# Ezreal11/EaBNet

Measured on AMD Instinct MI355X. Metric: enhanced frames/sec (16 kHz, 8-mic) at 1/2/4/8 MI355X; RTF per utterance, higher is better.
Workload: dtype f32; 1 GPU; BASELINE configs[1]/[2]: batch of 16 four-second 8-mic 16 kHz utterances per GPU, wave -> STFT+compress -> EaBNet.forward, inference, full hand-written HIP path; batch_per_gpu=16, global_batch=16, mics=8, frames_per_utt=401, freq_bins=161, parallelism=dp1 (independent shards, no collective), pipeline_depth=3

## Files before the change

### eabnet_amd/csrc/conv_gemm.hip

```cpp
#include "device.h"
#include <type_traits>

#define CG_THREADS 256

#define CG_PLAIN 0
#define CG_GLU 1
#define CG_DUAL 2
#define CG_PH2 3
#define CG_XFC 128

#define CG_PMAX 352

template <int MI, int NI, int KU, int MODE, bool PATCH, bool XFT>
struct CgSmem {
    static constexpr int BM = 64 * MI, BN = 64 * NI, LDK = 16 * KU + 4;
    static constexpr int NA = MODE == CG_DUAL ? 2 : 1;
    static constexpr int ATILE = BM * LDK;
    float a[PATCH ? CG_PMAX * LDK : NA * 2 * ATILE];
    float b[2][BN * LDK];
    float xft[2][CG_XFC][2];
    float xsl[2][CG_XFC];
    int dt[EAB_MAX_TAPS];
    int ioff[EAB_MAX_TAPS];
    int last;
    static constexpr int RW = MODE == CG_PH2 ? 2 : 1;
    __attribute__((aligned(16))) unsigned rtab_own[XFT ? BM * RW : 4];
    static_assert(XFT || sizeof(float) * 2 * CG_XFC * 2 >= sizeof(unsigned) * BM * RW, "row table inside xft");
};

__device__ __forceinline__ void cg_merge(float& n, float& mean, float& m2, float nb, float meanb, float m2b) {
    const float nt = n + nb;
    if (nt > 0.0f) {
        const float delta = meanb - mean;
        const float fb = nb / nt;
        mean = fmaf(delta, fb, mean);
        m2 = m2 + m2b + delta * delta * n * fb;
    }
    n = nt;
}

template <int MI, int NI, int KU, int MODE, int XF, bool VEC, int PREC, bool PATCH, bool WIDE = false>
__global__ __launch_bounds__(CG_THREADS, (MI == 2 && NI == 2 && KU == 1 && MODE == CG_GLU) ? 3 : (MODE == CG_PH2 ? 2 : 1)) void conv_gemm_kernel(const eab_conv_desc d) {
    static_assert(MODE != CG_PH2 || (PATCH && NI == 2), "phase-pair form: patch pipeline, one column block per phase and wave");
    static_assert(!PATCH || (KU == 1 && MODE != CG_DUAL && VEC), "patch mode: one unit per stage, single transform");
    constexpr bool H3 = PREC == EAB_PREC_F16X3;
    constexpr bool BF = PREC == EAB_PREC_BF16;
    constexpr bool PH2 = MODE == CG_PH2;
    constexpr bool GLU = MODE != CG_PLAIN;
    constexpr bool DUAL = MODE == CG_DUAL;
    using Smem = CgSmem<MI, NI, KU, MODE, PATCH, XF != EAB_XF_NONE>;
    constexpr int BM = Smem::BM, BN = Smem::BN, LDK = Smem::LDK;
    __shared__ __attribute__((aligned(16))) Smem sm;

    const int tid = threadIdx.x;
    const int lane = tid & 63, wave = tid >> 6;
    const int wm = wave >> 1, wn = wave & 1;
    const int li = lane & 31, lh = lane >> 5;

    const int t_lo = d.win.pos ? *d.win.pos : 0;
    int t_hi = d.win.pos ? (t_lo + d.win.count < d.T ? t_lo + d.win.count : d.T) : d.T;
    const int tiles_per_b = ((d.win.pos ? d.win.count : d.T) * d.No + BM - 1) / BM;
    unsigned vblk = blockIdx.x;
    if (gridDim.x >= 64) {
        const unsigned G = gridDim.x, G8 = G >> 3, rem = G & 7, xcd = vblk & 7, idx = vblk >> 3;
        vblk = xcd * G8 + (xcd < rem ? xcd : rem) + idx;
    }
    const int b = (int)(vblk / (unsigned)tiles_per_b);
    const int tile = (int)vblk - b * tiles_per_b;
    int t_src = d.T;
    if (d.win.lens) {
        t_src = min(t_src, d.win.lens[b]);
        t_hi = min(t_hi, t_src);
    }
    const int Q = t_hi * d.No;
    const int q0 = t_lo * d.No + tile * BM;
    const int n_blk = blockIdx.y * BN;
    const float inv_no = 1.0f / (float)d.No;

#pragma unroll
    for (int j = 0; j < EAB_MAX_TAPS; ++j)
        if (tid == j) {
            sm.dt[j] = d.dt[j];
            sm.ioff[j] = d.ioff[j];
        }

    const int Cout = d.Cout;
    const unsigned row_bytes = (unsigned)(d.Fout * Cout) * 4u, step_bytes = (unsigned)(d.ostride * Cout) * 4u;
    const unsigned phase_bytes = (unsigned)(d.ophase * Cout) * 4u, chan_bytes = (unsigned)Cout * 4u;
    unsigned* const rtab = XF != EAB_XF_NONE ? sm.rtab_own : reinterpret_cast<unsigned*>(&sm.xft[0][0][0]);
    if (tid < BM) {
        const int q = q0 + tid;
        const bool ok = q < Q;
        const int t = eab_div(ok ? q : 0, d.No, inv_no), o = (ok ? q : 0) - t * d.No;
        const unsigned off = ok ? (unsigned)t * row_bytes + (unsigned)o * step_bytes + phase_bytes : EAB_OOB;
        if constexpr (PH2)
            *reinterpret_cast<uint2*>(&rtab[2 * tid]) = make_uint2(off, (ok && 2 * o + 1 < d.Fout) ? off + chan_bytes : EAB_OOB);
        else
            rtab[tid] = off;
    }

    if (XF != EAB_XF_NONE) {
        const int k = tid >> 7, c = tid & (CG_XFC - 1);
        const int Ck = (k == 0 || DUAL) ? d.C0 : d.C1;
        const float* xfk = k == 0 ? d.xf0 : d.xf1;
        const float* slk = k == 0 ? d.slope0 : d.slope1;
        float sc = 1.0f, sh = 0.0f, sl = 1.0f;
        if (c < Ck) {
            if (d.fin_stats && k < d.fin_nsets) {
                const float* gm = k == 0 ? d.fin_gamma0 : d.fin_gamma1;
                const float* bt = k == 0 ? d.fin_beta0 : d.fin_beta1;
                double sn = 0.0, sm = 0.0, sq = 0.0;
                for (int t = 0; t < d.fin_tiles; ++t) {
                    const f32x4 v = *reinterpret_cast<const f32x4*>(
                        &d.fin_stats[((((size_t)b * d.fin_tiles + t) * d.fin_nsets + k) * d.C0 + c) * 4]);
                    const double n = (double)v[0], mu = (double)v[1];
                    sn += n;
                    sm = fma(n, mu, sm);
                    sq += fma(n * mu, mu, (double)v[2]);
                }
                const double mean = sn > 0.0 ? sm / sn : 0.0;
                double var = sn > 0.0 ? sq / sn - mean * mean : 0.0;
                if (var < 0.0) var = 0.0;
                const double scale = (double)gm[c] / sqrt(var + (double)d.fin_eps);
                sc = (float)scale;
                sh = (float)((double)bt[c] - mean * scale);
                sl = slk[c];
            } else if (xfk) {
                const float2 v = *reinterpret_cast<const float2*>(&xfk[((size_t)b * Ck + c) * 2]);
                sc = v.x;
                sh = v.y;
                sl = slk[c];
            }
        }
        sm.xft[k][c][0] = sc;
        sm.xft[k][c][1] = sh;
        sm.xsl[k][c] = sl;
    }

    const int Ctot = d.C0 + d.C1;
    const int UPT = (Ctot + 15) >> 4;
    const int NU = d.ntaps * UPT;
    static_assert(!WIDE || (PREC == EAB_PREC_BF16 && KU == 1 && VEC && !PATCH && XF == EAB_XF_NONE && MODE != CG_DUAL), "WIDE: see above");
    constexpr bool w0 = WIDE, w1 = WIDE;
    const int NS = (w0 || w1) ? d.ntaps * ((w0 ? d.C0 >> 5 : (d.C0 + 15) >> 4) + (d.C1 > 0 ? (w1 ? d.C1 >> 5 : (d.C1 + 15) >> 4) : 0))
                              : (NU + KU - 1) / KU;

    constexpr unsigned esz0 = WIDE ? 2u : 4u, esz1 = WIDE ? 2u : 4u;
    const unsigned bytes0 = (unsigned)d.T * d.Fin * d.C0 * esz0;
    const unsigned bytes1 = (unsigned)d.T * d.Fin * d.C1 * esz1;
    const __amdgpu_buffer_rsrc_t rs0 = __builtin_amdgcn_make_buffer_rsrc(
        const_cast<char*>(reinterpret_cast<const char*>(d.src0)) + (size_t)b * bytes0, 0, bytes0, 0x00020000);
    const __amdgpu_buffer_rsrc_t rs1 = __builtin_amdgcn_make_buffer_rsrc(
        const_cast<char*>(reinterpret_cast<const char*>(d.src1 ? d.src1 : d.src0)) + (d.src1 ? (size_t)b * bytes1 : 0), 0,
        d.src1 ? bytes1 : 0u, 0x00020000);

    const int srow = tid >> 2;
    const int skq = tid & 3;
    const float* wrow[NI];
#pragma unroll
    for (int p = 0; p < NI; ++p) wrow[p] = d.w + (size_t)(n_blk + srow + 64 * p) * d.Kpad + skq * 4;

    f32x16 acc[MI][NI];
#pragma unroll
    for (int mi = 0; mi < MI; ++mi)
#pragma unroll
        for (int ni = 0; ni < NI; ++ni)
#pragma unroll
            for (int r = 0; r < 16; ++r) acc[mi][ni][r] = 0.0f;

    auto lds_barrier = [] { asm volatile("s_waitcnt lgkmcnt(0)\n\ts_barrier" ::: "memory"); };

    __syncthreads();

    if (q0 < Q) {
    if constexpr (PATCH) {
        constexpr int PP = (CG_PMAX + 63) / 64;
        int dt_min = 0, io_min = 0, io_max = 0;
#pragma unroll
        for (int j = 0; j < EAB_MAX_TAPS; ++j)
            if (j < d.ntaps) {
                dt_min = d.dt[j] < dt_min ? d.dt[j] : dt_min;
                io_min = d.ioff[j] < io_min ? d.ioff[j] : io_min;
                io_max = d.ioff[j] > io_max ? d.ioff[j] : io_max;
            }
        const int halo_lo = -io_min;
        const int hi_need = (d.No - 1) * d.istride + io_max - (d.Fin - 1);
        const int Fp = d.Fin + halo_lo + (hi_need > 0 ? hi_need : 0);
        const float inv_fp = 1.0f / (float)Fp;
        const int t_first = eab_div(q0, d.No, inv_no);
        const int t_last = eab_div((q0 + BM < Q ? q0 + BM : (Q > q0 ? Q : q0 + 1)) - 1, d.No, inv_no);
        const int P = (t_last - t_first + 1 - dt_min) * Fp;

        const int d64 = eab_div(64, Fp, inv_fp), m64 = 64 - d64 * Fp;
        int p_tf[PP];
        bool p_ok[PP], p_all[PP];
        {
            const int tr = eab_div(srow, Fp, inv_fp);
            int f = srow - tr * Fp, t_in = t_first + dt_min + tr;
            int tf = t_in * d.Fin + f - halo_lo;
#pragma unroll
            for (int pp = 0; pp < PP; ++pp) {
                p_ok[pp] = p_all[pp] = false;
                p_tf[pp] = 0;
                if (64 * pp < P) {
                    p_ok[pp] = srow + 64 * pp < P && (unsigned)t_in < (unsigned)t_src && (unsigned)(f - halo_lo) < (unsigned)d.Fin;
                    if (XF != EAB_XF_NONE) p_all[pp] = __builtin_amdgcn_ballot_w64(p_ok[pp]) == __builtin_amdgcn_ballot_w64(true);
                    p_tf[pp] = tf;
                    f += m64;
                    t_in += d64;
                    tf += d64 * d.Fin + m64;
                    if (f >= Fp) {
                        f -= Fp;
                        ++t_in;
                        tf += d.Fin - Fp;
                    }
                }
            }
        }
        int fa[MI];
#pragma unroll
        for (int mi = 0; mi < MI; ++mi) {
            int q = q0 + (wm * MI + mi) * 32 + li;
            q = q < Q ? q : (Q > q0 ? Q - 1 : q0);
            const int t = eab_div(q, d.No, inv_no), o = q - t * d.No;
            fa[mi] = ((t - t_first - dt_min) * Fp + o * d.istride + halo_lo) * LDK + 4 * lh;
        }
        const int b_base = (wn * NI * 32 + li) * LDK + 4 * lh;

        f32x4 rp[PP];
        f32x4 rbw0[NI], rbw1[NI];
        int p_tc = 0;
        auto patch_fetch = [&](int chunk) {
            const int c0 = chunk << 4;
            const bool second = (d.C1 > 0) && (c0 >= d.C0);
            const int Cs = second ? d.C1 : d.C0;
            const int c = (second ? c0 - d.C0 : c0) + skq * 4;
            const bool cok = c < Cs;
            p_tc = ((second ? 1 : 0) << 8) | (cok ? c : 0);
#pragma unroll
            for (int pp = 0; pp < PP; ++pp) {
                if (64 * pp >= P) continue;
                const unsigned off = (p_ok[pp] && cok) ? (unsigned)((p_tf[pp] * Cs + c) * 4) : EAB_OOB;
                const u32x4 v = second ? __builtin_amdgcn_raw_buffer_load_b128(rs1, off, 0, 0)
                                       : __builtin_amdgcn_raw_buffer_load_b128(rs0, off, 0, 0);
                rp[pp] = __builtin_bit_cast(f32x4, v);
            }
        };
        auto patch_stash = [&]() {
            f32x4 sh01, sh23, sl;
            if (XF != EAB_XF_NONE) {
                const int cc = p_tc & 0xFF, tb = p_tc >> 8;
                sh01 = *reinterpret_cast<const f32x4*>(&sm.xft[tb][cc][0]);
                sh23 = *reinterpret_cast<const f32x4*>(&sm.xft[tb][cc + 2][0]);
                sl = *reinterpret_cast<const f32x4*>(&sm.xsl[tb][cc]);
            }
#pragma unroll
            for (int pp = 0; pp < PP; ++pp) {
                const int pidx = srow + 64 * pp;
                if (pidx >= CG_PMAX) continue;
                if (64 * pp >= P) continue;
                f32x4 v = rp[pp];
                if (XF != EAB_XF_NONE) {
                    const f32x4 x = eab_xform<XF>(v, sh01, sh23, sl);
                    v = x;
                    if (!p_all[pp]) {
                        asm volatile("; rim" ::: "memory");
                        v = p_ok[pp] ? x : f32x4{0.f, 0.f, 0.f, 0.f};
                    }
                }
                float* arow = &sm.a[pidx * LDK];
                if (BF) {
                    *reinterpret_cast<uint2*>(reinterpret_cast<char*>(arow) + skq * 8) = make_uint2(eab_bf2(v[0], v[1]), eab_bf2(v[2], v[3]));
                } else if (H3) {
                    unsigned h01, l01, h23, l23;
                    eab_split2(v[0], v[1], h01, l01);
                    eab_split2(v[2], v[3], h23, l23);
                    *reinterpret_cast<uint2*>(reinterpret_cast<char*>(arow) + skq * 8) = make_uint2(h01, h23);
                    *reinterpret_cast<uint2*>(reinterpret_cast<char*>(arow) + 32 + skq * 8) = make_uint2(l01, l23);
                } else {
                    *reinterpret_cast<f32x4*>(arow + skq * 4) = v;
                }
            }
        };
        auto b_fetch = [&](int u, f32x4 (&rbw)[NI]) {
            const int uu = u < NU ? u : 0;
#pragma unroll
            for (int p = 0; p < NI; ++p) rbw[p] = *reinterpret_cast<const f32x4*>(wrow[p] + (size_t)uu * 16);
        };
        auto b_stash = [&](int buf, const f32x4 (&rbw)[NI]) {
#pragma unroll
            for (int p = 0; p < NI; ++p) {
                float* brow = &sm.b[buf][(srow + 64 * p) * LDK];
                if (BF) {
                    *reinterpret_cast<uint2*>(reinterpret_cast<char*>(brow) + skq * 8) =
                        make_uint2(eab_bf2(rbw[p][0], rbw[p][1]), eab_bf2(rbw[p][2], rbw[p][3]));
                } else if (H3) {
                    const u32x4 w = __builtin_bit_cast(u32x4, rbw[p]);
                    *reinterpret_cast<uint2*>(reinterpret_cast<char*>(brow) + skq * 8) = make_uint2(w[0], w[1]);
                    *reinterpret_cast<uint2*>(reinterpret_cast<char*>(brow) + 32 + skq * 8) = make_uint2(w[2], w[3]);
                } else {
                    *reinterpret_cast<f32x4*>(brow + skq * 4) = rbw[p];
                }
            }
        };
        auto pcompute_n = [&](int cur, int tap, auto ne_c) {
            constexpr int NE = decltype(ne_c)::value;
            const int toff = (sm.dt[tap] * Fp + sm.ioff[tap]) * LDK;
            if (BF) {
                bf16x8 ab[MI], bb[NE];
#pragma unroll
                for (int mi = 0; mi < MI; ++mi) ab[mi] = *reinterpret_cast<const bf16x8*>(&sm.a[fa[mi] + toff]);
#pragma unroll
                for (int ni = 0; ni < NE; ++ni) bb[ni] = *reinterpret_cast<const bf16x8*>(&sm.b[cur][b_base + ni * 32 * LDK]);
#pragma unroll
                for (int mi = 0; mi < MI; ++mi)
#pragma unroll
                    for (int ni = 0; ni < NE; ++ni)
                        acc[mi][ni] = __builtin_amdgcn_mfma_f32_32x32x16_bf16(ab[mi], bb[ni], acc[mi][ni], 0, 0, 0);
            } else if (H3) {
                h16x8 ah[MI], al[MI], bh[NE], bl[NE];
#pragma unroll
                for (int mi = 0; mi < MI; ++mi) {
                    const char* pa = reinterpret_cast<const char*>(&sm.a[fa[mi] + toff]);
                    ah[mi] = *reinterpret_cast<const h16x8*>(pa);
                    al[mi] = *reinterpret_cast<const h16x8*>(pa + 32);
                }
#pragma unroll
                for (int ni = 0; ni < NE; ++ni) {
                    const char* pb = reinterpret_cast<const char*>(&sm.b[cur][b_base + ni * 32 * LDK]);
                    bh[ni] = *reinterpret_cast<const h16x8*>(pb);
                    bl[ni] = *reinterpret_cast<const h16x8*>(pb + 32);
                }
#pragma unroll
                for (int mi = 0; mi < MI; ++mi)
#pragma unroll
                    for (int ni = 0; ni < NE; ++ni) {
                        acc[mi][ni] = __builtin_amdgcn_mfma_f32_32x32x16_f16(al[mi], bh[ni], acc[mi][ni], 0, 0, 0);
                        acc[mi][ni] = __builtin_amdgcn_mfma_f32_32x32x16_f16(ah[mi], bl[ni], acc[mi][ni], 0, 0, 0);
                        acc[mi][ni] = __builtin_amdgcn_mfma_f32_32x32x16_f16(ah[mi], bh[ni], acc[mi][ni], 0, 0, 0);
                    }
            } else {
#pragma unroll
                for (int g = 0; g < 2; ++g) {
                    f32x4 af[MI], bf[NE];
#pragma unroll
                    for (int mi = 0; mi < MI; ++mi) af[mi] = *reinterpret_cast<const f32x4*>(&sm.a[fa[mi] + toff + g * 8]);
#pragma unroll
                    for (int ni = 0; ni < NE; ++ni)
                        bf[ni] = *reinterpret_cast<const f32x4*>(&sm.b[cur][b_base + ni * 32 * LDK + g * 8]);
#pragma unroll
                    for (int k = 0; k < 4; ++k)
#pragma unroll
                        for (int mi = 0; mi < MI; ++mi)
#pragma unroll
                            for (int ni = 0; ni < NE; ++ni)
                                acc[mi][ni] = __builtin_amdgcn_mfma_f32_32x32x2f32(af[mi][k], bf[ni][k], acc[mi][ni], 0, 0, 0);
                }
            }
        };
        const unsigned p2mask = PH2 ? (unsigned)d.p2_mask1 : ~0u;
        auto pcompute = [&](int cur, int tap) {
            if (PH2 && !((p2mask >> tap) & 1u)) pcompute_n(cur, tap, std::integral_constant<int, 1>{});
            else pcompute_n(cur, tap, std::integral_constant<int, NI>{});
        };

        patch_fetch(0);
        b_fetch(0, rbw0);
        patch_stash();
        b_stash(0, rbw0);
        b_fetch(1, rbw0);
        b_fetch(2, rbw1);
        lds_barrier();
        const int pre = d.ntaps >= 3 ? d.ntaps - 3 : 0;
        int chunk = 0, tap = 0;
        auto stage = [&](int u, int cur, f32x4 (&rnext)[NI]) {
            if (tap == pre && chunk + 1 < UPT) patch_fetch(chunk + 1);
            pcompute(cur, tap);
            if (u + 1 < NU) b_stash(cur ^ 1, rnext);
            b_fetch(u + 3, rnext);
            if (tap == d.ntaps - 1 && chunk + 1 < UPT) {
                lds_barrier();
                patch_stash();
            }
            lds_barrier();
            if (++tap == d.ntaps) { tap = 0; ++chunk; }
        };
        for (int u = 0; u < NU; u += 2) {
            stage(u, 0, rbw0);
            if (u + 1 < NU) stage(u + 1, 1, rbw1);
        }
        __syncthreads();
    } else {
    int a_t[MI], a_f0[MI], a_tf[MI];
    bool a_ok[MI];
#pragma unroll
    for (int p = 0; p < MI; ++p) {
        const int q = q0 + srow + 64 * p;
        a_ok[p] = q < Q;
        const int t = a_ok[p] ? eab_div(q, d.No, inv_no) : 0;
        const int o = a_ok[p] ? q - t * d.No : 0;
        a_t[p] = t;
        a_f0[p] = o * d.istride;
        a_tf[p] = t * d.Fin + o * d.istride;
    }
    struct Stage {
        f32x4 ra[KU][MI], rb[KU][NI];
        f32x4 rb2[BF ? NI : 1];
        int r_tc[KU];
        bool st_ok[KU][MI];
    };
    Stage sa;

    bool tap_ok[MI];
    unsigned tap_b0[MI], tap_b1[MI];
#pragma unroll
    for (int p = 0; p < MI; ++p) {
        tap_ok[p] = false;
        tap_b0[p] = tap_b1[p] = 0u;
    }
    int g_tap = -1, g_c0 = 0, g_w = 16;
    constexpr bool LEAN = KU == 1 && VEC && !DUAL;
    const __amdgpu_buffer_rsrc_t rsw = __builtin_amdgcn_make_buffer_rsrc(const_cast<float*>(d.w), 0, (unsigned)d.N * d.Kpad * 4u, 0x00020000);
    unsigned w_off[NI];
#pragma unroll
    for (int p = 0; p < NI; ++p) w_off[p] = (unsigned)((n_blk + srow + 64 * p) * d.Kpad + skq * 4) * 4u;
    auto fetch = [&](int stage, Stage& rg) {
        if constexpr (LEAN) {
            if (stage == 0) {
                g_tap = 0;
                g_c0 = 0;
            } else {
                g_c0 += g_w;
                if (g_c0 >= (UPT << 4)) {
                    g_c0 = 0;
                    ++g_tap;
                }
            }
            if (g_c0 == 0) {
                const int dt = sm.dt[g_tap], io = sm.ioff[g_tap];
#pragma unroll
                for (int p = 0; p < MI; ++p) {
                    const int tt = a_t[p] + dt, fi = a_f0[p] + io;
                    tap_ok[p] = a_ok[p] && tt >= 0 && tt < t_src && fi >= 0 && fi < d.Fin;
                    const unsigned pos = (unsigned)(a_tf[p] + dt * d.Fin + io);
                    tap_b0[p] = (pos * (unsigned)d.C0 + (unsigned)(skq * (w0 ? 8 : 4))) * esz0;
                    tap_b1[p] = (pos * (unsigned)d.C1 + (unsigned)(skq * (w1 ? 8 : 4))) * esz1;
                }
            }
            const bool second = (d.C1 > 0) && (g_c0 >= d.C0);
            const int Cs = second ? d.C1 : d.C0;
            const int cu = second ? g_c0 - d.C0 : g_c0;
            constexpr bool half = WIDE;
            g_w = half ? 32 : 16;
            const bool cok = cu + skq * (half ? 8 : 4) < Cs;
            const int k0 = g_tap * (UPT << 4) + g_c0;
#pragma unroll
            for (int p = 0; p < MI; ++p) {
                const bool ok = tap_ok[p] && cok;
                rg.st_ok[0][p] = ok;
                const unsigned off = ok ? (second ? tap_b1[p] : tap_b0[p]) : EAB_OOB;
                const u32x4 v = second ? __builtin_amdgcn_raw_buffer_load_b128(rs1, off, cu * (half ? 2 : 4), 0)
                                       : __builtin_amdgcn_raw_buffer_load_b128(rs0, off, cu * (half ? 2 : 4), 0);
                rg.ra[0][p] = __builtin_bit_cast(f32x4, v);
            }
            rg.r_tc[0] = ((half ? 1 : 0) << 9) | ((second ? 1 : 0) << 8) | cu;
#pragma unroll
            for (int p = 0; p < NI; ++p) {
                if constexpr (WIDE) {
                    rg.rb[0][p] = __builtin_bit_cast(f32x4, __builtin_amdgcn_raw_buffer_load_b128(rsw, w_off[p] + skq * 16, k0 * 4, 0));
                    if constexpr (BF)
                        rg.rb2[p] = __builtin_bit_cast(f32x4, __builtin_amdgcn_raw_buffer_load_b128(rsw, w_off[p] + skq * 16, k0 * 4 + 16, 0));
                } else {
                    rg.rb[0][p] = __builtin_bit_cast(f32x4, __builtin_amdgcn_raw_buffer_load_b128(rsw, w_off[p], k0 * 4, 0));
                }
            }
            return;
        }
#pragma unroll
        for (int ku = 0; ku < KU; ++ku) {
            const int u = stage * KU + ku;
            const bool live = u < NU;
            if (u == 0) {
                g_tap = 0;
                g_c0 = 0;
            } else if (live) {
                g_c0 += 16;
                if (g_c0 >= (UPT << 4)) {
                    g_c0 = 0;
                    ++g_tap;
                }
            }
            const int uu = live ? u : 0;
            const int c0 = live ? g_c0 : 0;
            if (live && c0 == 0) {
                const int dt = sm.dt[g_tap], io = sm.ioff[g_tap];
#pragma unroll
                for (int p = 0; p < MI; ++p) {
                    const int tt = a_t[p] + dt, fi = a_f0[p] + io;
                    tap_ok[p] = a_ok[p] && tt >= 0 && tt < t_src && fi >= 0 && fi < d.Fin;
                    const unsigned pos = (unsigned)(a_tf[p] + dt * d.Fin + io);
// ... 65 lines not shown
            for (int p = 0; p < MI; ++p) {
#pragma unroll
                for (int k = 0; k < (DUAL ? 2 : 1); ++k) {
                    f32x4 v = rg.ra[ku][p];
                    if (XF != EAB_XF_NONE) {
                        v = eab_xform<XF>(v, sh01[k], sh23[k], sl[k]);
                        if (!all_ok) {
                            asm volatile("; rim" ::: "memory");
                            v = rg.st_ok[ku][p] ? v : f32x4{0.f, 0.f, 0.f, 0.f};
                        }
                    }
                    float* arow = &sm.a[(k * 2 + buf) * Smem::ATILE + (srow + 64 * p) * LDK + ku * 16];
                    if (BF) {
                        constexpr bool half = WIDE;
                        if (half)
                            *reinterpret_cast<u32x4*>(reinterpret_cast<char*>(arow) + skq * 16) = __builtin_bit_cast(u32x4, v);
                        else
                            *reinterpret_cast<uint2*>(reinterpret_cast<char*>(arow) + skq * 8) = make_uint2(eab_bf2(v[0], v[1]), eab_bf2(v[2], v[3]));
                    } else if (H3) {
                        unsigned h01, l01, h23, l23;
                        eab_split2(v[0], v[1], h01, l01);
                        eab_split2(v[2], v[3], h23, l23);
                        *reinterpret_cast<uint2*>(reinterpret_cast<char*>(arow) + skq * 8) = make_uint2(h01, h23);
                        *reinterpret_cast<uint2*>(reinterpret_cast<char*>(arow) + 32 + skq * 8) = make_uint2(l01, l23);
                    } else {
                        *reinterpret_cast<f32x4*>(arow + skq * 4) = v;
                    }
                }
            }
#pragma unroll
            for (int p = 0; p < NI; ++p) {
                float* brow = &sm.b[buf][(srow + 64 * p) * LDK + ku * 16];
                if (BF) {
                    if constexpr (WIDE) {
                        const f32x4 r0 = rg.rb[ku][p], r1 = rg.rb2[BF ? p : 0];
                        *reinterpret_cast<u32x4*>(reinterpret_cast<char*>(brow) + skq * 16) =
                            u32x4{eab_bf2(r0[0], r0[1]), eab_bf2(r0[2], r0[3]), eab_bf2(r1[0], r1[1]), eab_bf2(r1[2], r1[3])};
                    } else {
                        *reinterpret_cast<uint2*>(reinterpret_cast<char*>(brow) + skq * 8) =
                            make_uint2(eab_bf2(rg.rb[ku][p][0], rg.rb[ku][p][1]), eab_bf2(rg.rb[ku][p][2], rg.rb[ku][p][3]));
                    }
                } else if (H3) {
                    const u32x4 w = __builtin_bit_cast(u32x4, rg.rb[ku][p]);
                    *reinterpret_cast<uint2*>(reinterpret_cast<char*>(brow) + skq * 8) = make_uint2(w[0], w[1]);
                    *reinterpret_cast<uint2*>(reinterpret_cast<char*>(brow) + 32 + skq * 8) = make_uint2(w[2], w[3]);
                } else {
                    *reinterpret_cast<f32x4*>(brow + skq * 4) = rg.rb[ku][p];
                }
            }
        }
    };

    fetch(0, sa);
    stash(0, sa);
    lds_barrier();

    const int a_base = (wm * MI * 32 + li) * LDK + 4 * lh;
    const int b_base = (wn * NI * 32 + li) * LDK + 4 * lh;

    auto compute = [&](int cur) {
        if (BF) {
#pragma unroll
            for (int ku = 0; ku < KU; ++ku) {
                bf16x8 ab[Smem::NA][MI], bb[NI];
#pragma unroll
                for (int k = 0; k < Smem::NA; ++k)
#pragma unroll
                    for (int mi = 0; mi < MI; ++mi)
                        ab[k][mi] = *reinterpret_cast<const bf16x8*>(&sm.a[(k * 2 + cur) * Smem::ATILE + a_base + mi * 32 * LDK + ku * 16]);
#pragma unroll
                for (int ni = 0; ni < NI; ++ni) bb[ni] = *reinterpret_cast<const bf16x8*>(&sm.b[cur][b_base + ni * 32 * LDK + ku * 16]);
#pragma unroll
                for (int mi = 0; mi < MI; ++mi)
#pragma unroll
                    for (int ni = 0; ni < NI; ++ni)
                        acc[mi][ni] = __builtin_amdgcn_mfma_f32_32x32x16_bf16(ab[DUAL ? ni : 0][mi], bb[ni], acc[mi][ni], 0, 0, 0);
            }
            if constexpr (WIDE) {
                bf16x8 ab[MI], bb[NI];
#pragma unroll
                for (int mi = 0; mi < MI; ++mi) ab[mi] = *reinterpret_cast<const bf16x8*>(&sm.a[cur * Smem::ATILE + a_base + mi * 32 * LDK + 8]);
#pragma unroll
                for (int ni = 0; ni < NI; ++ni) bb[ni] = *reinterpret_cast<const bf16x8*>(&sm.b[cur][b_base + ni * 32 * LDK + 8]);
#pragma unroll
                for (int mi = 0; mi < MI; ++mi)
#pragma unroll
                    for (int ni = 0; ni < NI; ++ni)
                        acc[mi][ni] = __builtin_amdgcn_mfma_f32_32x32x16_bf16(ab[mi], bb[ni], acc[mi][ni], 0, 0, 0);
            }
        } else if (H3) {
#pragma unroll
            for (int ku = 0; ku < KU; ++ku) {
                h16x8 ah[Smem::NA][MI], al[Smem::NA][MI], bh[NI], bl[NI];
#pragma unroll
                for (int k = 0; k < Smem::NA; ++k)
#pragma unroll
                    for (int mi = 0; mi < MI; ++mi) {
                        const char* pa = reinterpret_cast<const char*>(&sm.a[(k * 2 + cur) * Smem::ATILE + a_base + mi * 32 * LDK + ku * 16]);
                        ah[k][mi] = *reinterpret_cast<const h16x8*>(pa);
                        al[k][mi] = *reinterpret_cast<const h16x8*>(pa + 32);
                    }
#pragma unroll
                for (int ni = 0; ni < NI; ++ni) {
                    const char* pb = reinterpret_cast<const char*>(&sm.b[cur][b_base + ni * 32 * LDK + ku * 16]);
                    bh[ni] = *reinterpret_cast<const h16x8*>(pb);
                    bl[ni] = *reinterpret_cast<const h16x8*>(pb + 32);
// ... 356 lines not shown
                double sn = 0.0, sm_ = 0.0, sq = 0.0;
                if (slice < NSL) {
                    const float* p = d.stats + (((size_t)b * d.stat_tiles) * d.nsets + s) * Cout * 4 + (size_t)c * 4;
                    const size_t stride = (size_t)d.nsets * Cout * 4;
                    for (int t = slice; t < d.stat_tiles; t += NSL) {
                        const f32x4 v = *reinterpret_cast<const f32x4*>(p + (size_t)t * stride);
                        const double n = (double)v[0], mu = (double)v[1];
                        sn += n;
                        sm_ = fma(n, mu, sm_);
                        sq += fma(n * mu, mu, (double)v[2]);
                    }
                    dred[(0 * NSL + slice) * nch + e] = sn;
                    dred[(1 * NSL + slice) * nch + e] = sm_;
                    dred[(2 * NSL + slice) * nch + e] = sq;
                }
                __syncthreads();
                if (slice == 0) {
                    sn = sm_ = sq = 0.0;
                    for (int k = 0; k < NSL; ++k) {
                        sn += dred[(0 * NSL + k) * nch + e];
                        sm_ += dred[(1 * NSL + k) * nch + e];
                        sq += dred[(2 * NSL + k) * nch + e];
                    }
                    const double mean = sn > 0.0 ? sm_ / sn : 0.0;
                    double var = sn > 0.0 ? sq / sn - mean * mean : 0.0;
                    if (var < 0.0) var = 0.0;
                    const float* gm = s == 0 ? d.fz_gamma0 : d.fz_gamma1;
                    const float* bt = s == 0 ? d.fz_beta0 : d.fz_beta1;
                    float* xf = s == 0 ? d.fz_xf0 : d.fz_xf1;
                    const double scale = (double)gm[c] / sqrt(var + (double)d.fz_eps);
                    *reinterpret_cast<float2*>(&xf[((size_t)b * Cout + c) * 2]) = make_float2((float)scale, (float)((double)bt[c] - mean * scale));
                }
                if (tid == 0) d.fz_counter[b] = 0;
            }
        }
    }
}

extern "C" int eab_conv_tiles(int T, int No, int bm) {
    if (T <= 0 || No <= 0 || (bm != 16 && bm != 32 && bm != 64 && bm != 128)) return -1;
    long long q = (long long)T * No;
    return (int)((q + bm - 1) / bm);
}

int eab_conv_st(const eab_conv_desc* d, hipStream_t s);

template <int MI, int NI, int KU, int MODE, int XF, bool VEC>
static int cg_launch(const eab_conv_desc* d, hipStream_t s) {
    constexpr int BM = 64 * MI, BN = 64 * NI;
    const int tiles = eab_conv_tiles(d->win.pos ? d->win.count : d->T, d->No, BM);
    dim3 grid((unsigned)(d->B * tiles), (unsigned)(d->N / BN));
    constexpr bool can_patch = KU == 1 && MODE != CG_DUAL && VEC && XF != EAB_XF_PRELU_NORM;
    if (d->korder == EAB_KORDER_CHUNK) {
        if constexpr (can_patch) {
            if (d->precision == EAB_PREC_F16X3)
                hipLaunchKernelGGL((conv_gemm_kernel<MI, NI, 1, MODE, XF, true, EAB_PREC_F16X3, true>), grid,
                                   dim3(CG_THREADS), 0, s, *d);
            else if (d->precision == EAB_PREC_BF16)
                hipLaunchKernelGGL((conv_gemm_kernel<MI, NI, 1, MODE, XF, true, EAB_PREC_BF16, true>), grid,
                                   dim3(CG_THREADS), 0, s, *d);
            else
                hipLaunchKernelGGL((conv_gemm_kernel<MI, NI, 1, MODE, XF, true, EAB_PREC_F32, true>), grid,
                                   dim3(CG_THREADS), 0, s, *d);
            EAB_RETURN_LAUNCH_STATUS();
        } else {
            return EAB_EUNSUPPORTED;
        }
    }
    if constexpr (MODE == CG_PH2) {
        return EAB_EUNSUPPORTED;
    } else {
    if (d->precision == EAB_PREC_F16X3) {
        if constexpr (VEC)
            hipLaunchKernelGGL((conv_gemm_kernel<MI, NI, KU, MODE, XF, VEC, EAB_PREC_F16X3, false>), grid,
                               dim3(CG_THREADS), 0, s, *d);
        else
            return EAB_EUNSUPPORTED;
    } else if (d->precision == EAB_PREC_BF16) {
        if constexpr (VEC) {
            if (d->src_bf16) {
                if constexpr (KU == 1 && XF == EAB_XF_NONE && MODE != CG_DUAL)
                    hipLaunchKernelGGL((conv_gemm_kernel<MI, NI, KU, MODE, XF, VEC, EAB_PREC_BF16, false, true>), grid,
                                       dim3(CG_THREADS), 0, s, *d);
                else
                    return EAB_EUNSUPPORTED;
            } else {
                hipLaunchKernelGGL((conv_gemm_kernel<MI, NI, KU, MODE, XF, VEC, EAB_PREC_BF16, false>), grid,
                                   dim3(CG_THREADS), 0, s, *d);
            }
        } else {
            return EAB_EUNSUPPORTED;
        }
    } else {
        hipLaunchKernelGGL((conv_gemm_kernel<MI, NI, KU, MODE, XF, VEC, EAB_PREC_F32, false>), grid, dim3(CG_THREADS), 0,
                           s, *d);
    }
    EAB_RETURN_LAUNCH_STATUS();
    }
}

static long long cg_patch_positions(const eab_conv_desc* d) {
    int dt_min = 0, io_min = 0, io_max = 0;
    for (int j = 0; j < d->ntaps; ++j) {
        dt_min = d->dt[j] < dt_min ? d->dt[j] : dt_min;
        io_min = d->ioff[j] < io_min ? d->ioff[j] : io_min;
        io_max = d->ioff[j] > io_max ? d->ioff[j] : io_max;
    }
    const int hi_need = (d->No - 1) * d->istride + io_max - (d->Fin - 1);
    const long long Fp = d->Fin - io_min + (hi_need > 0 ? hi_need : 0);
    const long long rows = (d->bm - 1) / d->No + 2 - dt_min;
    return rows * Fp;
}

template <int MI, int NI, int MODE, int XF, bool VEC>
static int cg_pick_ku(const eab_conv_desc* d, hipStream_t s, int ku) {
    if (ku == 4) {
        if constexpr (MI == 1 && MODE != CG_GLU && VEC) return cg_launch<MI, NI, 4, MODE, XF, VEC>(d, s);
        return EAB_EUNSUPPORTED;
    }
    if (ku == 2) {
        if constexpr (VEC && MODE != CG_DUAL) return cg_launch<MI, NI, 2, MODE, XF, VEC>(d, s);
        return EAB_EUNSUPPORTED;
// ... 41 lines not shown
    const long long per_b = (long long)d->T * d->Fin * (d->C0 > d->C1 ? d->C0 : d->C1) * 4;
    EAB_CHECK_ARG(per_b < (1ll << 31) && (long long)d->T * d->Fout * d->Cout * 4 < (1ll << 31));
    EAB_CHECK_ARG((long long)d->T * d->No < (1ll << 22));
    EAB_CHECK_ARG(d->xf_mode >= EAB_XF_NONE && d->xf_mode <= EAB_XF_PRELU_NORM);
    if (d->src_bf16) {
        EAB_CHECK_ARG((d->src_bf16 & ~3) == 0 && d->precision == EAB_PREC_BF16 && d->korder == EAB_KORDER_TAP);
        EAB_CHECK_ARG(d->xf_mode == EAB_XF_NONE && d->fin_stats == nullptr && d->Fin > 1 && d->epi != EAB_EPI_DUALGATE);
        EAB_CHECK_ARG(d->C0 % 16 == 0 && d->C1 % 16 == 0 && (!(d->src_bf16 & 2) || d->src1));
        EAB_CHECK_ARG((!(d->src_bf16 & 1) || d->C0 % 32 == 0) && (!(d->src_bf16 & 2) || d->C1 % 32 == 0));
        EAB_CHECK_ARG(d->src_bf16 == (d->src1 ? 3 : 1));
    }
    const bool fin = d->fin_stats != nullptr;
    if (fin) {
        EAB_CHECK_ARG(d->xf_mode != EAB_XF_NONE && !d->xf0 && !d->xf1 && d->C1 == 0);
        EAB_CHECK_ARG(d->fin_tiles > 0 && d->fin_tiles <= 64 && d->fin_count > 0);
        EAB_CHECK_ARG(d->fin_nsets == (dual ? 2 : 1) || (!dual && d->fin_nsets == 2));
        EAB_CHECK_ARG(d->fin_gamma0 && d->fin_beta0 && d->slope0);
        EAB_CHECK_ARG(!dual || (d->fin_gamma1 && d->fin_beta1 && d->slope1));
    }
    if (d->xf_mode != EAB_XF_NONE) {
        EAB_CHECK_ARG(fin || (d->xf0 == nullptr) == (d->slope0 == nullptr));
        EAB_CHECK_ARG(fin || dual || (d->xf1 == nullptr) == (d->slope1 == nullptr));
    }
    if (dual) {
        EAB_CHECK_ARG(d->C1 == 0 && d->xf_mode != EAB_XF_NONE && d->slope0 && d->slope1);
        EAB_CHECK_ARG(fin || (d->xf0 && d->xf1));
    }
    EAB_CHECK_ARG((d->epi != EAB_EPI_MULSIG && d->epi != EAB_EPI_ADD) || d->aux);
    EAB_CHECK_ARG(d->nsets >= 0 && d->nsets <= 2 && (d->nsets == 0) == (d->stats == nullptr));
    EAB_CHECK_ARG(d->korder == EAB_KORDER_FRAG ? (d->bm == 16 || d->bm == 32 || d->bm == 64) : (d->bm == 64 || d->bm == 128));
    if (d->fz_counter) {
        EAB_CHECK_ARG(d->stats && d->nsets >= 1 && d->nsets * d->Cout <= CG_THREADS && d->win.pos == nullptr);
        EAB_CHECK_ARG(d->fz_gamma0 && d->fz_beta0 && d->fz_xf0 && (d->nsets == 1 || (d->fz_gamma1 && d->fz_beta1 && d->fz_xf1)));
    }
    if (d->stats) {
        const int tiles = eab_conv_tiles(d->T, d->No, d->bm) + (d->ph1_No > 0 ? eab_conv_tiles(d->T, d->ph1_No, d->bm) : 0);
        EAB_CHECK_ARG(d->stat_tile0 >= 0 && d->stat_tile0 + tiles <= d->stat_tiles);
    }
    EAB_CHECK_ARG((long long)d->B * (eab_conv_tiles(d->T, d->No, d->bm) + (d->ph1_No > 0 ? eab_conv_tiles(d->T, d->ph1_No, d->bm) : 0)) < (1ll << 31));
    hipStream_t s = eab_stream(stream);
    if (d->korder == EAB_KORDER_FRAG) return eab_conv_st(d, s);
    const int mi = d->bm / 64;
    const bool vec = (d->C0 % 4 == 0) && (d->C1 % 4 == 0);
    const bool has_xf = d->xf_mode != EAB_XF_NONE && (d->xf0 || d->xf1 || fin);
    const int xf = has_xf ? d->xf_mode : EAB_XF_NONE;
    if (xf != EAB_XF_NONE)
        EAB_CHECK_ARG(d->C0 <= CG_XFC && d->C1 <= CG_XFC && vec);
    int ku = (mi == 1 && !glu && vec && d->Fin == 1) ? 4 : 1;
    if (d->korder == EAB_KORDER_CHUNK) ku = 1;
    if (ku == 4 && !(mi == 1 && !glu && vec)) ku = 1;
    if (ku == 2 && (!vec || dual)) ku = 1;
    if (ph2) {
        if (!vec || xf == EAB_XF_PRELU_NORM) return EAB_EUNSUPPORTED;
        if (xf == EAB_XF_NORM_PRELU)
            return mi == 2 ? cg_launch<2, 2, 1, CG_PH2, EAB_XF_NORM_PRELU, true>(d, s) : cg_launch<1, 2, 1, CG_PH2, EAB_XF_NORM_PRELU, true>(d, s);
        return mi == 2 ? cg_launch<2, 2, 1, CG_PH2, EAB_XF_NONE, true>(d, s) : cg_launch<1, 2, 1, CG_PH2, EAB_XF_NONE, true>(d, s);
    }
    if (dual) {
        if (d->N != 128 || mi != 1 || xf != EAB_XF_PRELU_NORM) return EAB_EUNSUPPORTED;
        return cg_pick_ku<1, 2, CG_DUAL, EAB_XF_PRELU_NORM, true>(d, s, ku == 2 ? 1 : ku);
    }
    if (glu) {
        if (d->N % 128 != 0 || xf == EAB_XF_PRELU_NORM) return EAB_EUNSUPPORTED;
        if (!vec) return mi == 2 ? cg_pick_ku<2, 2, CG_GLU, 0, false>(d, s, 1) : cg_pick_ku<1, 2, CG_GLU, 0, false>(d, s, 1);
        if (xf == EAB_XF_NORM_PRELU)
            return mi == 2 ? cg_pick_ku<2, 2, CG_GLU, EAB_XF_NORM_PRELU, true>(d, s, ku)
                           : cg_pick_ku<1, 2, CG_GLU, EAB_XF_NORM_PRELU, true>(d, s, ku);
        return mi == 2 ? cg_pick_ku<2, 2, CG_GLU, 0, true>(d, s, ku) : cg_pick_ku<1, 2, CG_GLU, 0, true>(d, s, ku);
    }
    if (!vec) return EAB_EUNSUPPORTED;
#define CG_DISPATCH_XF(MI_, NI_)                                                           \
    (xf == EAB_XF_NONE        ? cg_pick_ku<MI_, NI_, CG_PLAIN, EAB_XF_NONE, true>(d, s, ku) \
     : xf == EAB_XF_NORM_PRELU ? cg_pick_ku<MI_, NI_, CG_PLAIN, EAB_XF_NORM_PRELU, true>(d, s, ku) \
                               : cg_pick_ku<MI_, NI_, CG_PLAIN, EAB_XF_PRELU_NORM, true>(d, s, ku))
    if (d->N % 128 == 0) return mi == 2 ? CG_DISPATCH_XF(2, 2) : CG_DISPATCH_XF(1, 2);
    if (d->N % 64 == 0) return mi == 2 ? CG_DISPATCH_XF(2, 1) : CG_DISPATCH_XF(1, 1);
#undef CG_DISPATCH_XF
    return EAB_EUNSUPPORTED;
}

extern "C" int eab_conv_bf16(const eab_conv_desc* d, eab_stream_t stream) {
    EAB_CHECK_ARG(d);
    eab_conv_desc dd = *d;
    dd.precision = EAB_PREC_BF16;
    return eab_conv_f32(&dd, stream);
}
```

### eabnet_amd/program.py

```python
from __future__ import annotations

import functools
import os
from dataclasses import dataclass, field, replace
from typing import Dict, List, Optional, Sequence, Tuple

import numpy as np

from ._lib import MAX_TAPS
from .spec import GagConfig, NetConfig, gag_param_specs, gate_key, param_specs, unet_decoder_layers, unet_encoder_layers

XF_NONE, XF_NORM_PRELU, XF_PRELU_NORM = 0, 1, 2
EPI_LINEAR, EPI_GLU, EPI_RELU, EPI_MULSIG, EPI_ADD, EPI_DUALGATE, EPI_PHASE2 = 0, 1, 2, 3, 4, 5, 6
OP_CONV, OP_IN_FINALIZE, OP_NORM_ACT, OP_LSTM64, OP_BFW_FS, OP_MEMSET0, OP_GAG_PACK, OP_GAG_CRM = 1, 2, 3, 4, 5, 6, 7, 8
OP_CONV_CHAIN = 9
(OP_GATHER, OP_IN_STATS, OP_TR_NORM_ACT, OP_NORM_BWD, OP_GLU_BWD, OP_GATE_FWD, OP_GATE_BWD, OP_ADD, OP_RELU_BWD, OP_COLSUM,
 OP_FILTER_SUM, OP_FS_BWD, OP_LN_FWD, OP_LN_BWD, OP_LSTM_TRAIN, OP_LSTM_BWD) = range(16, 32)
OP_WGRAD = 32
OP_CLN_STATS, OP_CLN_APPLY, OP_GATE_ROWS = 33, 34, 35
OP_GAG_CRM_BWD, OP_CLN_BWD = 36, 37
OP_CLN_STEP = 38
NB_SUMS_ZEROED = 0x100
NB_SUM_COPIES = 8
STORE_BF16 = 0x200
ACT_SIGMOID, ACT_TANH, ACT_RELU = 0, 1, 2
GAG_PRE_LD = 324
GAG_LIN_LD = 192
PREC_F32, PREC_F16X3, PREC_BF16 = 0, 1, 2
PREC_CODE = {"f32": PREC_F32, "f16x3": PREC_F16X3, "bf16": PREC_BF16}
KORDER_TAP, KORDER_CHUNK, KORDER_FRAG = 0, 1, 2
ST_GLU_KMAX = 512
PATCH_MAX = 352
EPS_IN = 1e-5
EPS_LN = 1e-5
ALIGN = 64
CUS = 256


@dataclass(frozen=True)
class Ref:
    arena: str
    off: int = 0


@dataclass
class Act:
    ref: Ref
    F: int
    C: int
    xf: Optional[Ref] = None
    slope: Optional[Ref] = None
    mode: int = XF_NONE
    raw: bool = False


@dataclass
class ConvOp:
    src0: Ref
    src1: Optional[Ref]
    xf0: Optional[Ref]
    xf1: Optional[Ref]
    slope0: Optional[Ref]
    slope1: Optional[Ref]
    C0: int
    C1: int
    xf_mode: int
    w: Ref
    bias: Optional[Ref]
    N: int
    Kpad: int
    B: int
    T: int
    Fin: int
    Fout: int
    No: int
    ostride: int
    ophase: int
    istride: int
    dt: List[int]
    ioff: List[int]
    epi: int
    aux: Optional[Ref]
    dst: Ref
    dst_acc: Optional[Ref]
    Cout: int
# ... 306 lines not shown
        for p in range(g.istride):
            tp = [j for j in range(g.ntaps) if (g.ioff[j] - p) % g.istride == 0]
            No = (g.Fin - p + g.istride - 1) // g.istride
            if No > 0 and tp:
                out.append(Geometry(g.Fout, g.Fin, No, g.istride, p, 1, tuple(-g.dt[j] for j in tp),
                                    tuple(-(g.ioff[j] - p) // g.istride for j in tp), tuple(g.taps[j] for j in tp)))
        return out


def tcm_taps(kd: int, dilation: int, causal: bool) -> List[int]:
    span = (kd - 1) * dilation
    lead = span if causal else span // 2
    return [j * dilation - lead for j in range(kd)]


@dataclass(frozen=True)
class Stats:
    ref: Optional[Ref]
    tiles: int
    nsets: int = 1
    slopes: Tuple[Optional[Ref], Optional[Ref]] = (None, None)
    tile0: int = 0


def conv_launch(name: str, B: int, T: int, srcs: Sequence, w: Ref, bias: Optional[Ref], geom: Geometry, *, N: int, epi: int,
                dst: Ref, bm: int, stats: Optional[Stats] = None, ph1: Optional[Tuple[Ref, Geometry]] = None, **fields) -> ConvOp:
    s0, s1 = srcs[0], (srcs[1] if len(srcs) > 1 else None)
    C0, C1 = s0.C, (s1.C if s1 else 0)
    assert geom.Fin == s0.F and geom.ntaps <= MAX_TAPS
    st = stats if stats is not None and stats.ref is not None else Stats(None, 0, 0)
    kw = {**dict(xf0=None, xf1=None, slope0=None, slope1=None, xf_mode=XF_NONE, aux=None, dst_acc=None), **fields}
    if ph1 is not None:
        w1, g1 = ph1
        assert (g1.Fin, g1.Fout, g1.ostride, g1.istride) == (geom.Fin, geom.Fout, geom.ostride, geom.istride) and g1.ntaps <= geom.ntaps
        kw.update(ph1_w=w1, ph1_No=g1.No, ph1_ophase=g1.ophase, ph1_Kpad=g1.kpad(C0 + C1), ph1_dt=list(g1.dt), ph1_ioff=list(g1.ioff))
    return ConvOp(src0=s0.ref, src1=s1.ref if s1 else None, C0=C0, C1=C1, w=w, bias=bias, N=N, Kpad=geom.kpad(C0 + C1), B=B, T=T,
                  Fin=geom.Fin, Fout=geom.Fout, No=geom.No, ostride=geom.ostride, ophase=geom.ophase, istride=geom.istride,
                  dt=list(geom.dt), ioff=list(geom.ioff), epi=epi, dst=dst,
                  Cout=N // 2 if epi in (EPI_GLU, EPI_DUALGATE, EPI_PHASE2) else N, stats=st.ref, nsets=st.nsets,
                  stat_slope0=st.slopes[0], stat_slope1=st.slopes[1], stat_tiles=st.tiles, stat_tile0=st.tile0, bm=bm, name=name, **kw)


def conv_tiles(T: int, No: int, bm: int) -> int:
    return (T * No + bm - 1) // bm


def patch_positions(bm: int, No: int, Fin: int, istride: int, dt, ioff) -> int:
    dt_min, io_min, io_max = min(0, min(dt)), min(0, min(ioff)), max(0, max(ioff))
    hi_need = (No - 1) * istride + io_max - (Fin - 1)
    Fp = Fin - io_min + max(hi_need, 0)
    return ((bm - 1) // No + 2 - dt_min) * Fp


def glu_row_order(N: int) -> np.ndarray:
    r = np.arange(N)
    return (r % 64 // 32) * (N // 2) + (r // 64) * 32 + r % 32


def unit_rows(N: int, glu: bool, frag: bool = False) -> Tuple[np.ndarray, int]:
    return (glu_row_order(N) if glu and not frag else np.arange(N)), (N // 2 if glu else N)


def pack_taps(w_nck: np.ndarray, taps_k: Sequence[int]) -> np.ndarray:
    N, C, _ = w_nck.shape
    upt = (C + 15) // 16
    idx = np.issubdtype(w_nck.dtype, np.integer)
    out = np.full((N, len(taps_k), upt * 16), -1 if idx else 0, dtype=w_nck.dtype if idx else np.float32)
    for j, k in enumerate(taps_k):
        out[:, j, :C] = w_nck[:, :, k]
    return out.reshape(N, -1)


def pack_f16x3(wp: np.ndarray) -> np.ndarray:
    N, K = wp.shape
    assert K % 4 == 0
    if np.abs(wp).max(initial=0.0) >= 65504.0:
        raise ValueError("f16x3 precision needs |weight| < 65504")
    hi = wp.astype(np.float16)
    lo = (wp - hi.astype(np.float32)).astype(np.float16)
    out = np.empty((N, K // 4, 8), dtype=np.float16)
    out[:, :, :4] = hi.reshape(N, K // 4, 4)
    out[:, :, 4:] = lo.reshape(N, K // 4, 4)
    return np.ascontiguousarray(out).view(np.float32).reshape(N, K)


def _frag_index(N: int, K: int):
    nb, m2, lane, j = np.meshgrid(np.arange(N // 16), np.arange(K // 16), np.arange(64), np.arange(4), indexing="ij")
    return nb * 16 + (lane & 15), 16 * m2 + 8 * (j >> 1) + 2 * (lane >> 4) + (j & 1)


def frag_row_order(N: int, dual: bool) -> np.ndarray:
    r = np.arange(N)
    if not dual:
        return r
    return ((r // 16) % 2) * (N // 2) + (r // 32) * 16 + r % 16


def pack_frag(wp: np.ndarray, dual: bool = False) -> np.ndarray:
    N, K = wp.shape
    assert N % 16 == 0 and K % 16 == 0
    n, k = _frag_index(N, K)
    return np.ascontiguousarray(wp[frag_row_order(N, dual)][n, k],
                                dtype=wp.dtype if np.issubdtype(wp.dtype, np.integer) else np.float32).reshape(-1)


def unpack_frag(flat: np.ndarray, N: int, K: int, dual: bool = False) -> np.ndarray:
# ... 780 lines not shown
```

Before: 999,100 frames/s.

## Add short-patch phase-pair conv variant and overlap transform setup with first fetch

Adds a CG_PH2S mode for f32 phase-pair convs whose patch fits in 256 positions. It uses a smaller LDS patch buffer, which should allow more resident blocks, and a dedicated compute routine that loads A fragments once per tap and skips the second column block when the phase mask says so. It also moves the per-channel norm/PReLU transform setup so it runs after the first global fetches are issued, hiding its latency instead of waiting behind a full barrier. Tap address setup is pulled into a helper that takes the first tap directly from the descriptor. The extra template instantiations add code size, and the reordered barriers are a correctness risk.

```diff
diff --git a/eabnet_amd/csrc/conv_gemm.hip b/eabnet_amd/csrc/conv_gemm.hip
--- a/eabnet_amd/csrc/conv_gemm.hip
+++ b/eabnet_amd/csrc/conv_gemm.hip
@@ -7,23 +7,28 @@
 #define CG_GLU 1
 #define CG_DUAL 2
 #define CG_PH2 3
+#define CG_PH2S 4
 #define CG_XFC 128
 
 #define CG_PMAX 352
+#define CG_PSHORT 256
+
+constexpr bool cg_ph2(int mode) { return mode == CG_PH2 || mode == CG_PH2S; }
 
 template <int MI, int NI, int KU, int MODE, bool PATCH, bool XFT>
 struct CgSmem {
     static constexpr int BM = 64 * MI, BN = 64 * NI, LDK = 16 * KU + 4;
     static constexpr int NA = MODE == CG_DUAL ? 2 : 1;
     static constexpr int ATILE = BM * LDK;
-    float a[PATCH ? CG_PMAX * LDK : NA * 2 * ATILE];
+    static constexpr int PMAX = MODE == CG_PH2S ? CG_PSHORT : CG_PMAX;
+    float a[PATCH ? PMAX * LDK : NA * 2 * ATILE];
     float b[2][BN * LDK];
     float xft[2][CG_XFC][2];
     float xsl[2][CG_XFC];
     int dt[EAB_MAX_TAPS];
     int ioff[EAB_MAX_TAPS];
     int last;
-    static constexpr int RW = MODE == CG_PH2 ? 2 : 1;
+    static constexpr int RW = cg_ph2(MODE) ? 2 : 1;
     __attribute__((aligned(16))) unsigned rtab_own[XFT ? BM * RW : 4];
     static_assert(XFT || sizeof(float) * 2 * CG_XFC * 2 >= sizeof(unsigned) * BM * RW, "row table inside xft");
 };
@@ -40,12 +45,12 @@
 }
 
 template <int MI, int NI, int KU, int MODE, int XF, bool VEC, int PREC, bool PATCH, bool WIDE = false>
-__global__ __launch_bounds__(CG_THREADS, (MI == 2 && NI == 2 && KU == 1 && MODE == CG_GLU) ? 3 : (MODE == CG_PH2 ? 2 : 1)) void conv_gemm_kernel(const eab_conv_desc d) {
-    static_assert(MODE != CG_PH2 || (PATCH && NI == 2), "phase-pair form: patch pipeline, one column block per phase and wave");
+__global__ __launch_bounds__(CG_THREADS, (MI == 2 && NI == 2 && KU == 1 && MODE == CG_GLU) ? 3 : (cg_ph2(MODE) ? 2 : 1)) void conv_gemm_kernel(const eab_conv_desc d) {
+    static_assert(!cg_ph2(MODE) || (PATCH && NI == 2), "phase-pair form: patch pipeline, one column block per phase and wave");
     static_assert(!PATCH || (KU == 1 && MODE != CG_DUAL && VEC), "patch mode: one unit per stage, single transform");
     constexpr bool H3 = PREC == EAB_PREC_F16X3;
     constexpr bool BF = PREC == EAB_PREC_BF16;
-    constexpr bool PH2 = MODE == CG_PH2;
+    constexpr bool PH2 = cg_ph2(MODE);
     constexpr bool GLU = MODE != CG_PLAIN;
     constexpr bool DUAL = MODE == CG_DUAL;
     using Smem = CgSmem<MI, NI, KU, MODE, PATCH, XF != EAB_XF_NONE>;
@@ -99,42 +104,9 @@
             rtab[tid] = off;
     }
 
-    if (XF != EAB_XF_NONE) {
-        const int k = tid >> 7, c = tid & (CG_XFC - 1);
-        const int Ck = (k == 0 || DUAL) ? d.C0 : d.C1;
-        const float* xfk = k == 0 ? d.xf0 : d.xf1;
-        const float* slk = k == 0 ? d.slope0 : d.slope1;
-        float sc = 1.0f, sh = 0.0f, sl = 1.0f;
-        if (c < Ck) {
-            if (d.fin_stats && k < d.fin_nsets) {
-                const float* gm = k == 0 ? d.fin_gamma0 : d.fin_gamma1;
-                const float* bt = k == 0 ? d.fin_beta0 : d.fin_beta1;
-                double sn = 0.0, sm = 0.0, sq = 0.0;
-                for (int t = 0; t < d.fin_tiles; ++t) {
-                    const f32x4 v = *reinterpret_cast<const f32x4*>(
-                        &d.fin_stats[((((size_t)b * d.fin_tiles + t) * d.fin_nsets + k) * d.C0 + c) * 4]);
-                    const double n = (double)v[0], mu = (double)v[1];
-                    sn += n;
-                    sm = fma(n, mu, sm);
-                    sq += fma(n * mu, mu, (double)v[2]);
-                }
-                const double mean = sn > 0.0 ? sm / sn : 0.0;
-                double var = sn > 0.0 ? sq / sn - mean * mean : 0.0;
-                if (var < 0.0) var = 0.0;
-                const double scale = (double)gm[c] / sqrt(var + (double)d.fin_eps);
-                sc = (float)scale;
-                sh = (float)((double)bt[c] - mean * scale);
-                sl = slk[c];
-            } else if (xfk) {
-                const float2 v = *reinterpret_cast<const float2*>(&xfk[((size_t)b * Ck + c) * 2]);
-                sc = v.x;
-                sh = v.y;
-                sl = slk[c];
-            }
-        }
-        sm.xft[k][c][0] = sc;
-        sm.xft[k][c][1] = sh;
-        sm.xsl[k][c] = sl;
+    constexpr bool EARLY = PATCH || (KU == 1 && VEC && !DUAL);
+    if constexpr (!EARLY) {
+#include "conv_gemm_xf.inc"
     }
 
     const int Ctot = d.C0 + d.C1;
@@ -170,11 +142,12 @@
 
     auto lds_barrier = [] { asm volatile("s_waitcnt lgkmcnt(0)\n\ts_barrier" ::: "memory"); };
 
-    __syncthreads();
+    if constexpr (!EARLY) __syncthreads();
+    else if (q0 >= Q) lds_barrier();
 
     if (q0 < Q) {
     if constexpr (PATCH) {
-        constexpr int PP = (CG_PMAX + 63) / 64;
+        constexpr int PP = (Smem::PMAX + 63) / 64;
         int dt_min = 0, io_min = 0, io_max = 0;
 #pragma unroll
         for (int j = 0; j < EAB_MAX_TAPS; ++j)
@@ -257,7 +230,7 @@
 #pragma unroll
             for (int pp = 0; pp < PP; ++pp) {
                 const int pidx = srow + 64 * pp;
-                if (pidx >= CG_PMAX) continue;
+                if (pidx >= Smem::PMAX) continue;
                 if (64 * pp >= P) continue;
                 f32x4 v = rp[pp];
                 if (XF != EAB_XF_NONE) {
@@ -359,13 +332,40 @@
             }
         };
         const unsigned p2mask = PH2 ? (unsigned)d.p2_mask1 : ~0u;
+        auto pcompute_ph2 = [&](int cur, int tap) {
+            const int toff = (sm.dt[tap] * Fp + sm.ioff[tap]) * LDK;
+            f32x4 af[2][MI];
+#pragma unroll
+            for (int g = 0; g < 2; ++g)
+#pragma unroll
+                for (int mi = 0; mi < MI; ++mi) af[g][mi] = *reinterpret_cast<const f32x4*>(&sm.a[fa[mi] + toff + g * 8]);
+            auto block = [&](auto ni_c) {
+                constexpr int ni = decltype(ni_c)::value;
+#pragma unroll
+                for (int g = 0; g < 2; ++g) {
+                    const f32x4 bf = *reinterpret_cast<const f32x4*>(&sm.b[cur][b_base + ni * 32 * LDK + g * 8]);
+#pragma unroll
+                    for (int k = 0; k < 4; ++k)
+#pragma unroll
+                        for (int mi = 0; mi < MI; ++mi)
+                            acc[mi][ni] = __builtin_amdgcn_mfma_f32_32x32x2f32(af[g][mi][k], bf[k], acc[mi][ni], 0, 0, 0);
+                }
+            };
+            block(std::integral_constant<int, 0>{});
+            if ((p2mask >> tap) & 1u) block(std::integral_constant<int, NI - 1>{});
+        };
         auto pcompute = [&](int cur, int tap) {
-            if (PH2 && !((p2mask >> tap) & 1u)) pcompute_n(cur, tap, std::integral_constant<int, 1>{});
+            if constexpr (PH2 && !BF && !H3) pcompute_ph2(cur, tap);
+            else if (PH2 && !((p2mask >> tap) & 1u)) pcompute_n(cur, tap, std::integral_constant<int, 1>{});
             else pcompute_n(cur, tap, std::integral_constant<int, NI>{});
         };
 
         patch_fetch(0);
         b_fetch(0, rbw0);
+        {
+#include "conv_gemm_xf.inc"
+        }
+        lds_barrier();
         patch_stash();
         b_stash(0, rbw0);
         b_fetch(1, rbw0);
@@ -424,28 +424,29 @@
     unsigned w_off[NI];
 #pragma unroll
     for (int p = 0; p < NI; ++p) w_off[p] = (unsigned)((n_blk + srow + 64 * p) * d.Kpad + skq * 4) * 4u;
+    auto tap_enter = [&](int dt, int io) {
+#pragma unroll
+        for (int p = 0; p < MI; ++p) {
+            const int tt = a_t[p] + dt, fi = a_f0[p] + io;
+            tap_ok[p] = a_ok[p] && tt >= 0 && tt < t_src && fi >= 0 && fi < d.Fin;
+            const unsigned pos = (unsigned)(a_tf[p] + dt * d.Fin + io);
+            tap_b0[p] = (pos * (unsigned)d.C0 + (unsigned)(skq * (w0 ? 8 : 4))) * esz0;
+            tap_b1[p] = (pos * (unsigned)d.C1 + (unsigned)(skq * (w1 ? 8 : 4))) * esz1;
+        }
+    };
     auto fetch = [&](int stage, Stage& rg) {
         if constexpr (LEAN) {
             if (stage == 0) {
                 g_tap = 0;
                 g_c0 = 0;
+                tap_enter(d.dt[0], d.ioff[0]);
             } else {
                 g_c0 += g_w;
                 if (g_c0 >= (UPT << 4)) {
                     g_c0 = 0;
                     ++g_tap;
                 }
-            }
-            if (g_c0 == 0) {
-                const int dt = sm.dt[g_tap], io = sm.ioff[g_tap];
-#pragma unroll
-                for (int p = 0; p < MI; ++p) {
-                    const int tt = a_t[p] + dt, fi = a_f0[p] + io;
-                    tap_ok[p] = a_ok[p] && tt >= 0 && tt < t_src && fi >= 0 && fi < d.Fin;
-                    const unsigned pos = (unsigned)(a_tf[p] + dt * d.Fin + io);
-                    tap_b0[p] = (pos * (unsigned)d.C0 + (unsigned)(skq * (w0 ? 8 : 4))) * esz0;
-                    tap_b1[p] = (pos * (unsigned)d.C1 + (unsigned)(skq * (w1 ? 8 : 4))) * esz1;
-                }
+                if (g_c0 == 0) tap_enter(sm.dt[g_tap], sm.ioff[g_tap]);
             }
             const bool second = (d.C1 > 0) && (g_c0 >= d.C0);
             const int Cs = second ? d.C1 : d.C0;
@@ -617,6 +618,10 @@
     };
 
     fetch(0, sa);
+    if constexpr (EARLY) {
+#include "conv_gemm_xf.inc"
+        lds_barrier();
+    }
     stash(0, sa);
     lds_barrier();
 
@@ -1079,7 +1084,10 @@
     dim3 grid((unsigned)(d->B * tiles), (unsigned)(d->N / BN));
     constexpr bool can_patch = KU == 1 && MODE != CG_DUAL && VEC && XF != EAB_XF_PRELU_NORM;
     if (d->korder == EAB_KORDER_CHUNK) {
-        if constexpr (can_patch) {
+        if constexpr (MODE == CG_PH2S) {
+            hipLaunchKernelGGL((conv_gemm_kernel<MI, NI, 1, MODE, XF, true, EAB_PREC_F32, true>), grid, dim3(CG_THREADS), 0, s, *d);
+            EAB_RETURN_LAUNCH_STATUS();
+        } else if constexpr (can_patch) {
             if (d->precision == EAB_PREC_F16X3)
                 hipLaunchKernelGGL((conv_gemm_kernel<MI, NI, 1, MODE, XF, true, EAB_PREC_F16X3, true>), grid,
                                    dim3(CG_THREADS), 0, s, *d);
@@ -1094,7 +1102,7 @@
             return EAB_EUNSUPPORTED;
         }
     }
-    if constexpr (MODE == CG_PH2) {
+    if constexpr (cg_ph2(MODE)) {
         return EAB_EUNSUPPORTED;
     } else {
     if (d->precision == EAB_PREC_F16X3) {
@@ -1242,6 +1250,11 @@
     if (ku == 2 && (!vec || dual)) ku = 1;
     if (ph2) {
         if (!vec || xf == EAB_XF_PRELU_NORM) return EAB_EUNSUPPORTED;
+        if (d->precision == EAB_PREC_F32 && cg_patch_positions(d) <= CG_PSHORT) {
+            if (xf == EAB_XF_NORM_PRELU)
+                return mi == 2 ? cg_launch<2, 2, 1, CG_PH2S, EAB_XF_NORM_PRELU, true>(d, s) : cg_launch<1, 2, 1, CG_PH2S, EAB_XF_NORM_PRELU, true>(d, s);
+            return mi == 2 ? cg_launch<2, 2, 1, CG_PH2S, EAB_XF_NONE, true>(d, s) : cg_launch<1, 2, 1, CG_PH2S, EAB_XF_NONE, true>(d, s);
+        }
         if (xf == EAB_XF_NORM_PRELU)
             return mi == 2 ? cg_launch<2, 2, 1, CG_PH2, EAB_XF_NORM_PRELU, true>(d, s) : cg_launch<1, 2, 1, CG_PH2, EAB_XF_NORM_PRELU, true>(d, s);
         return mi == 2 ? cg_launch<2, 2, 1, CG_PH2, EAB_XF_NONE, true>(d, s) : cg_launch<1, 2, 1, CG_PH2, EAB_XF_NONE, true>(d, s);
diff --git a/eabnet_amd/csrc/conv_gemm_xf.inc b/eabnet_amd/csrc/conv_gemm_xf.inc
--- /dev/null
+++ b/eabnet_amd/csrc/conv_gemm_xf.inc
@@ -0,0 +1,37 @@
+    if (XF != EAB_XF_NONE) {
+        const int k = tid >> 7, c = tid & (CG_XFC - 1);
+        const int Ck = (k == 0 || DUAL) ? d.C0 : d.C1;
+        const float* xfk = k == 0 ? d.xf0 : d.xf1;
+        const float* slk = k == 0 ? d.slope0 : d.slope1;
+        float sc = 1.0f, sh = 0.0f, sl = 1.0f;
+        if (c < Ck) {
+            if (d.fin_stats && k < d.fin_nsets) {
+                const float* gm = k == 0 ? d.fin_gamma0 : d.fin_gamma1;
+                const float* bt = k == 0 ? d.fin_beta0 : d.fin_beta1;
+                double sn = 0.0, sm = 0.0, sq = 0.0;
+                for (int t = 0; t < d.fin_tiles; ++t) {
+                    const f32x4 v = *reinterpret_cast<const f32x4*>(
+                        &d.fin_stats[((((size_t)b * d.fin_tiles + t) * d.fin_nsets + k) * d.C0 + c) * 4]);
+                    const double n = (double)v[0], mu = (double)v[1];
+                    sn += n;
+                    sm = fma(n, mu, sm);
+                    sq += fma(n * mu, mu, (double)v[2]);
+                }
+                const double mean = sn > 0.0 ? sm / sn : 0.0;
+                double var = sn > 0.0 ? sq / sn - mean * mean : 0.0;
+                if (var < 0.0) var = 0.0;
+                const double scale = (double)gm[c] / sqrt(var + (double)d.fin_eps);
+                sc = (float)scale;
+                sh = (float)((double)bt[c] - mean * scale);
+                sl = slk[c];
+            } else if (xfk) {
+                const float2 v = *reinterpret_cast<const float2*>(&xfk[((size_t)b * Ck + c) * 2]);
+                sc = v.x;
+                sh = v.y;
+                sl = slk[c];
+            }
+        }
+        sm.xft[k][c][0] = sc;
+        sm.xft[k][c][1] = sh;
+        sm.xsl[k][c] = sl;
+    }
diff --git a/eabnet_amd/program.py b/eabnet_amd/program.py
--- a/eabnet_amd/program.py
+++ b/eabnet_amd/program.py
@@ -31,6 +31,7 @@
 KORDER_TAP, KORDER_CHUNK, KORDER_FRAG = 0, 1, 2
 ST_GLU_KMAX = 512
 PATCH_MAX = 352
+PATCH_SHORT = 256
 EPS_IN = 1e-5
 EPS_LN = 1e-5
 ALIGN = 64
@@ -443,6 +444,13 @@
     return ((bm - 1) // No + 2 - dt_min) * Fp
 
 
+def phase_pair_passes(op: "ConvOp") -> int:
+    assert op.epi == EPI_PHASE2 and op.korder == KORDER_CHUNK
+    P = patch_positions(op.bm, op.No, op.Fin, op.istride, op.dt, op.ioff)
+    assert P <= PATCH_MAX
+    return 4 if op.precision == PREC_F32 and P <= PATCH_SHORT else 6
+
+
 def glu_row_order(N: int) -> np.ndarray:
     r = np.arange(N)
     return (r % 64 // 32) * (N // 2) + (r // 64) * 32 + r % 32
```

Result: faster. 1.019 million frames/s (median of 6 runs) (+2.0%).
